# moberweger/deep-prior-pp

Measured on AMD Instinct MI355X. Metric: depth-crops/sec (NYU ResNet50 bs128) 1/2/4/8 GPU; mean 3D joint err (mm), higher is better.
Workload: dtype f32; 1 GPU; NYU posereg_embedding ResNet (type 0, 30-D PCA prior) train step: fused augment + fwd + bwd + ADAM, bs128/GPU fp32, 128x128x1 crops; global_batch=128, parallelism=dp1, augment=True, augment_pipelined=True, bn=local per-GPU batch statistics, launch_mode=native

## Files before the change

### deep-prior-pp_amd/csrc/bn.hip

```cpp
#include "dpp_common.h"

namespace {

constexpr int MAXQ = 256;

template <class TX>
__global__ __launch_bounds__(DPP_THREADS) void bn_stats_partial_kernel(const TX* __restrict__ X, int M, int C,
                                                                       int rpb, float* __restrict__ partial) {
    __shared__ float s_mean[DPP_THREADS * 4];
    __shared__ float s_m2[DPP_THREADS * 4];
    __shared__ float s_n[DPP_THREADS];
    const int Q = C >> 2;
    const int RP = DPP_THREADS / Q;
    const int tid = threadIdx.x;
    const int q = tid % Q, rr = tid / Q;
    const int r_begin = blockIdx.x * rpb;
    const int r_end = (r_begin + rpb < M) ? r_begin + rpb : M;
    float4 K = make_float4(0.f, 0.f, 0.f, 0.f), s1 = K, s2 = K;
    int n = 0;
    if (rr < RP) {
        for (int r = r_begin + rr; r < r_end; r += RP) {
            float4 v = dpp_ld4(X + (size_t)r * C + q * 4);
            if (n == 0) K = v;
            float dx = v.x - K.x, dy = v.y - K.y, dz = v.z - K.z, dw = v.w - K.w;
// ... 15 lines not shown
        for (int j = 0; j < RP; ++j) {
            int t = j * Q + cq;
            double nb = (double)s_n[t];
            if (nb == 0.0) continue;
            double mb = (double)s_mean[t * 4 + ce], m2b = (double)s_m2[t * 4 + ce];
            double delta = mb - mean, tot = cn + nb;
            mean += delta * nb / tot;
            m2 += m2b + delta * delta * cn * nb / tot;
            cn = tot;
        }
        partial[dpp_partial_index(0, c, blockIdx.x, C, gridDim.x)] = (float)mean;
        partial[dpp_partial_index(1, c, blockIdx.x, C, gridDim.x)] = (float)m2;
    }
}

__device__ __forceinline__ double wave_allsum(double v) {
    for (int o = 1; o < DPP_WAVE; o <<= 1) v += __shfl_xor(v, o);
    return v;
}

template <int WPC>
__device__ __forceinline__ double group_allsum(double v, double* slot) {
    v = wave_allsum(v);
    if (WPC == 1) return v;
    const int wave = threadIdx.x >> 6;
    if ((threadIdx.x & 63) == 0) slot[wave] = v;
    __syncthreads();
    return ((slot[0] + slot[1]) + slot[2]) + slot[3];
}

template <int U, int WPC>
__global__ __launch_bounds__(DPP_THREADS) void bn_finalize_kernel(const float* __restrict__ partial, int nbs, int nseg, int M, int rpb,
                                                                  int C, const float* __restrict__ gamma, float eps,
                                                                  float* __restrict__ mean_o, float* __restrict__ inv_std_o,
                                                                  float* __restrict__ scale_o, float* __restrict__ run_mean,
                                                                  float* __restrict__ run_inv_std, float alpha) {
    dpp_kernarg_warm<96>();
    __shared__ double slot_a[4], slot_b[4];
    constexpr int GT = DPP_WAVE * WPC;
    const int lane = threadIdx.x % GT;
    const int c = blockIdx.x * (DPP_THREADS / GT) + threadIdx.x / GT;
    const int cc = c < C ? c : C - 1;
    const bool upd = alpha > 0.0f && run_mean != nullptr;
    const float gam = gamma[cc];
    const float rm_old = (upd ? run_mean : gamma)[cc], ri_old = (upd ? run_inv_std : gamma)[cc];
    const int Mseg = M / nseg;
    auto rows_of = [&](int bi) { return (bi * rpb + rpb <= Mseg) ? rpb : (Mseg - bi * rpb); };
    const bool one_sweep = nseg == 1 && nbs <= GT * U;
    float pm0[U], pq0[U];
    if (one_sweep) {
        const float* pm_row = partial + dpp_partial_index(0, cc, 0, C, nbs);
        const float* pq_row = partial + dpp_partial_index(1, cc, 0, C, nbs);
        const float K = pm_row[0];
#pragma unroll
        for (int u = 0; u < U; ++u) {
            const int b = lane + u * GT;
            const int bb = b < nbs ? b : nbs - 1;
            pm0[u] = pm_row[bb];
            pq0[u] = pq_row[bb];
        }
        double s1 = 0.0, s2 = 0.0;
#pragma unroll
        for (int u = 0; u < U; ++u) {
            const int b = lane + u * GT;
            if (b < nbs) {
                const double d = (double)pm0[u] - (double)K, nb_ = (double)rows_of(b);
                s1 += nb_ * d;
                s2 += (double)pq0[u] + nb_ * d * d;
            }
        }
        s1 = group_allsum<WPC>(s1, slot_a);
        s2 = group_allsum<WPC>(s2, slot_b);
        if (lane != 0 || c >= C) return;
        const double mean1 = (double)K + s1 / (double)M;
        const double var1 = (s2 - s1 * s1 / (double)M) / (double)M;
        const float meanf = (float)mean1;
        const float inv_std = (float)(1.0 / sqrt((var1 > 0.0 ? var1 : 0.0) + (double)eps));
        mean_o[c] = meanf;
        inv_std_o[c] = inv_std;
        scale_o[c] = gam * inv_std;
        if (upd) {
            const float oma = 1.0f - alpha;
            run_mean[c] = oma * rm_old + alpha * meanf;
            run_inv_std[c] = oma * ri_old + alpha * inv_std;
        }
        return;
    }
    double snm = 0.0;
    for (int seg = 0; seg < nseg; ++seg) {
        const float* pm_row = partial + (size_t)seg * 2 * C * nbs + dpp_partial_index(0, cc, 0, C, nbs);
        const float* pq_row = partial + (size_t)seg * 2 * C * nbs + dpp_partial_index(1, cc, 0, C, nbs);
        for (int b0 = lane; b0 < nbs; b0 += GT * U) {
            float pm[U];
#pragma unroll
            for (int u = 0; u < U; ++u) {
                const int b = b0 + u * GT;
                const int bb = b < nbs ? b : nbs - 1;
                pm[u] = pm_row[bb];
            }
#pragma unroll
// ... 443 lines not shown
```

### deep-prior-pp_amd/csrc/gemm.hip

```cpp
#include "gemm_kernels.h"

namespace {

__global__ __launch_bounds__(DPP_THREADS) void reduce_partials_kernel(const float* __restrict__ partial, int nz, int n,
                                                                      const float* __restrict__ bias, int nbias,
                                                                      float* __restrict__ out, int ZL) {
    __shared__ float red[DPP_THREADS];
    const int CB = DPP_THREADS / ZL;
    const int col = threadIdx.x % CB, zl = threadIdx.x / CB;
    for (int i0 = blockIdx.x * CB; i0 < n; i0 += gridDim.x * CB) {
        int i = i0 + col;
        float s = 0.0f;
        if (i < n)
            for (int z = zl; z < nz; z += ZL) s += partial[(size_t)z * n + i];
        if (ZL > 1) {
            red[threadIdx.x] = s;
            __syncthreads();
            if (zl == 0) {
                for (int j = 1; j < ZL; ++j) s += red[j * CB + col];
            }
        }
        if (zl == 0 && i < n) {
            if (bias) s += bias[i % nbias];
            out[i] = s;
// ... 79 lines not shown

bool aligned16(const void* p) { return (reinterpret_cast<uintptr_t>(p) & 15) == 0; }

static int gemm_prepare(const dpp_gemm_desc* dp, GemmArgs& ga) {
    if (!dp || !dp->A || !dp->B || dp->M <= 0 || dp->N <= 0 || dp->K <= 0) return DPP_E_BADARG;
    ga.d = *dp;
    ga.prof = dpp_prof_buffer;
    dpp_gemm_desc& d = ga.d;
    if (d.splitk < 1) d.splitk = 1;
    if (d.splitk > 1 && !d.partial) return DPP_E_BADARG;
    if (d.splitk > 1 && (d.epi.stats || d.epi.bn_x)) return DPP_E_BADARG;
    if (d.epi.bn_x && !(d.epi.bn_mean && d.epi.bn_inv_std && d.epi.bn_scale && d.epi.bn_beta && d.epi.bn_partial)) return DPP_E_BADARG;
    if (d.splitk == 1 && !d.C) return DPP_E_BADARG;
    if (d.actA.mode && d.actA.cmod <= 0) return DPP_E_BADARG;
    if (d.actB.mode && d.actB.cmod <= 0) return DPP_E_BADARG;
    ga.vecA = aligned16(d.A) && (d.lda % 4 == 0);
    if (d.actB.mode & 4) return DPP_E_UNSUPPORTED;
    if (d.actA.mode & 4) {
        if (d.actA.mode != 4 || d.variant == 1 || !d.actA.x2 || !d.actA.aux || !d.actA.mean || !d.actA.scale || !d.actA.beta) return DPP_E_BADARG;
        ga.vecA = ga.vecA && aligned16(d.actA.x2) && aligned16(d.actA.out);
        if (d.actA.out && (!d.a_kc || d.splitk != 1 || d.mapA.s != 1)) return DPP_E_UNSUPPORTED;
        if (!(aligned16(d.actA.mean) && aligned16(d.actA.scale) && aligned16(d.actA.beta) && aligned16(d.actA.aux))) return DPP_E_BADARG;
    }
    ga.vecB = aligned16(d.B) && (d.ldb % 4 == 0);
    if (d.store & ~(DPP_ST_A | DPP_ST_B | DPP_ST_C | DPP_ST_BNX)) return DPP_E_BADARG;
    if (d.precision != 0 && d.precision != 1) return DPP_E_BADARG;
    if (d.precision == 1 && (d.variant == 1 || (d.actA.mode & 4))) return DPP_E_UNSUPPORTED;
    if ((d.store & DPP_ST_A) && (!ga.vecA || (d.actA.mode & 4))) return DPP_E_UNSUPPORTED;
    if ((d.store & DPP_ST_B) && !ga.vecB) return DPP_E_UNSUPPORTED;
    if ((d.store & (DPP_ST_C | DPP_ST_BNX)) && d.splitk != 1) return DPP_E_UNSUPPORTED;
// ... 97 lines not shown
```

### deep-prior-pp_amd/csrc/gemm_expand.hip

```cpp
#include "gemm_args.h"

namespace {

template <int KT, bool BKC, bool IT2, bool ACT, bool RES, bool BNB, bool LZ = false, bool PB = false, bool ST = false>
__global__ __launch_bounds__(DPP_THREADS) DPP_WAVES_PER_EU(1, 2) void gemm_expand_kernel(GemmArgs ga, int rpw) {
    static_assert(!PB || ((KT % 32 == 0 || KT == 16) && !LZ), "bf16 MFMA operands: whole 32-deep steps, or K = 16 with a zero upper half");
    dpp_kernarg_warm<sizeof(GemmArgs)>();
    const dpp_gemm_desc& d = ga.d;
    constexpr int KL = KT / 4, KV = KL / 4;
    constexpr int RT = 2, RI = 16 * RT;
    const int lane = threadIdx.x & 63, l15 = lane & 15, kq = lane >> 4;
    const int NG = d.N >> 6, nblk = d.M / rpw;
    const int gw = blockIdx.x * 4 + (threadIdx.x >> 6);
    if (gw >= NG * nblk) return;
    const int cg = gw % NG, rblk = gw / NG;
    const int n0 = cg * 64 + 4 * l15;
    const int wrow0 = rblk * rpw, iters = rpw / RI;
    const dpp_epilogue& ep = d.epi;
    const int modeA = ACT ? d.actA.mode : 0;
    const bool relu_mask = BNB && ep.bn_relu != 0;
    const bool a16 = ST && !LZ && ga.shA != 0, c16 = ST && (d.store & DPP_ST_C) != 0, x16 = ST && (d.store & DPP_ST_BNX) != 0;
    dpp_stamp(ga.prof, 0);

    float bw[4][KL];
    if (BKC) {
#pragma unroll
        for (int ct = 0; ct < 4; ++ct)
#pragma unroll
            for (int j = 0; j < KV; ++j) {
// ... 33 lines not shown
                    if (LZ) g.a2[rt][j] = *reinterpret_cast<const float4*>(d.actA.x2 + oa + 4 * j);
                }
            }
        }
#pragma unroll
        for (int rt = 0; rt < RT; ++rt)
#pragma unroll
            for (int r = 0; r < 4; ++r) {
                const size_t o = (size_t)(r0 + rt * 16 + kq * 4 + r) * d.ldc + n0;
                if (RES) g.res[rt][r] = c16 ? dpp_raw8(d.residual + (o >> 1)) : *reinterpret_cast<const float4*>(d.residual + o);
                if (BNB) g.bx[rt][r] = x16 ? dpp_raw8(ep.bn_x + (o >> 1)) : *reinterpret_cast<const float4*>(ep.bn_x + o);
            }
    };
    Regs g0, g1;
    fetch(g0, 0);
    float4 mu[KV], sc[KV], be[KV], ax[LZ ? KV : 1];
#pragma unroll
    for (int j = 0; j < KV; ++j) {
        mu[j] = sc[j] = be[j] = make_float4(0.f, 0.f, 0.f, 0.f);
        if (LZ || (modeA & 2)) {
            mu[j] = *reinterpret_cast<const float4*>(d.actA.mean + kq * KL + 4 * j);
            sc[j] = *reinterpret_cast<const float4*>(d.actA.scale + kq * KL + 4 * j);
            be[j] = *reinterpret_cast<const float4*>(d.actA.beta + kq * KL + 4 * j);
        }
        if (LZ) ax[j] = *reinterpret_cast<const float4*>(d.actA.aux + kq * KL + 4 * j);
    }
    const bool lz_store = LZ && d.actA.out != nullptr && cg == 0;
    float4 cbias = make_float4(0.f, 0.f, 0.f, 0.f), cmean = cbias, cscale = cbias, cbeta = cbias, cistd = cbias;
    if (d.bias) cbias = *reinterpret_cast<const float4*>(d.bias + n0);
    if (BNB) {
        cmean = *reinterpret_cast<const float4*>(ep.bn_mean + n0); cscale = *reinterpret_cast<const float4*>(ep.bn_scale + n0);
        cbeta = *reinterpret_cast<const float4*>(ep.bn_beta + n0); cistd = *reinterpret_cast<const float4*>(ep.bn_inv_std + n0);
    }
    dpp_stamp(ga.prof, 1);

    float sx[4] = {0.f, 0.f, 0.f, 0.f}, sy[4] = {0.f, 0.f, 0.f, 0.f};
    float rmean[4] = {0.f, 0.f, 0.f, 0.f}, rm2[4] = {0.f, 0.f, 0.f, 0.f};
    const bool want_stats = ep.stats != nullptr;
    auto colsum = [&](float (&s)[4]) {
#pragma unroll
        for (int j = 0; j < 4; ++j) { s[j] += __shfl_xor(s[j], 16); s[j] += __shfl_xor(s[j], 32); }
    };

    auto step = [&](Regs& g, int it) {
// ... 155 lines not shown
}

}

int dpp_gemm_expand_rows(const dpp_gemm_desc& d, const GemmArgs& ga) {
    if ((d.store & DPP_ST_B) || (d.store && (d.actA.mode & 4))) return 0;
    if (!d.a_kc || d.splitk != 1 || !d.C || !ga.vecA || !ga.vecB || !ga.wide) return 0;
    if (d.K != 16 && d.K != 32 && d.K != 64) return 0;
    if (d.N % 64 || d.M % 32) return 0;
    if (d.mapA.s != 1 || d.mapB.s != 1 || d.mapC.s != 1 || d.actB.mode != 0) return 0;
    if (d.actA.mode != 0 && d.actA.cmod < d.K) return 0;
    if (d.epi.stats && d.epi.bn_x) return 0;
    if (d.b_kc ? (d.epi.bn_x != nullptr || (d.actA.mode & 4)) : (d.actA.mode != 0 && d.actA.mode != 4)) return 0;
    if (d.actA.mode == 4 && d.actA.out && d.lda != d.K) return 0;
    if (d.precision != 0 && (d.precision != 1 || (d.actA.mode & 4))) return 0;
    int rpw = d.bm;
    if (rpw <= 0) rpw = d.M >= 65536 ? 128 : (d.M >= 16384 ? 64 : 32);
    if (rpw % 32 || d.M % rpw) return 0;
    return rpw;
}

namespace {

template <int KT>
int launch_expand(const GemmArgs& ga, int rpw, hipStream_t st) {
    const dpp_gemm_desc& d = ga.d;
    const int waves = (d.M / rpw) * (d.N / 64);
    const dim3 grid(dpp_cdiv(waves, 4));
    const bool it2 = rpw > 32, act = d.actA.mode != 0, res = d.residual != nullptr, bnb = d.epi.bn_x != nullptr, lz = d.actA.mode == 4;
    const bool pb = d.precision == 1;
    const bool stg = d.store != 0;
#define DPP_EXS(K_, I_, A_, R_, B_, L_, P_, S_) DPP_LAUNCH((gemm_expand_kernel<KT, K_, I_, A_, R_, B_, L_, P_, S_>), grid, dim3(DPP_THREADS), 0, st, ga, rpw)
#define DPP_EX(K_, I_, A_, R_, B_, L_, P_) do { if (!(L_) && stg) DPP_EXS(K_, I_, A_, R_, B_, L_, P_, !(L_)); else DPP_EXS(K_, I_, A_, R_, B_, L_, P_, false); } while (0)
#define DPP_EX_P(K_, I_, A_, R_, B_) do { if (pb) { DPP_EX(K_, I_, A_, R_, B_, false, true); break; } \
                                          DPP_EX(K_, I_, A_, R_, B_, false, false); } while (0)
#define DPP_EX_I(K_, A_, R_, B_, L_) do { if (L_) { if (it2) DPP_EX(K_, true, A_, R_, B_, true, false); else DPP_EX(K_, false, A_, R_, B_, true, false); } \
                                          else if (it2) DPP_EX_P(K_, true, A_, R_, B_); else DPP_EX_P(K_, false, A_, R_, B_); } while (0)
#define DPP_EX_R(K_, A_, B_, L_) do { if (res) DPP_EX_I(K_, A_, true, B_, L_); else DPP_EX_I(K_, A_, false, B_, L_); } while (0)
    if (d.b_kc) {
        if (act) DPP_EX_R(true, true, false, false); else DPP_EX_R(true, false, false, false);
    } else if (lz) {
        if (bnb) DPP_EX_R(false, false, true, true); else DPP_EX_R(false, false, false, true);
    } else {
        if (bnb) DPP_EX_R(false, false, true, false); else DPP_EX_R(false, false, false, false);
    }
#undef DPP_EX_P
// ... 14 lines not shown
```

### deep-prior-pp_amd/hipdp/engine.py

```python
import os
from ctypes import c_int as C_int

import numpy as np

from . import evalfuse, layout, ops
from . import heuristics as hz
from .lib import Act, RowMap
from .ops import Plan
from .runtime import default_runtime
from .backward import BackwardMixin
from .store import BNState, ParamStore, TensorV, View, _collect, _dedupe_specs, _layer_kind, _pad4, _param_specs, bf16_bits_to_f32, get_store


class CompiledNet(BackwardMixin):
    def __init__(self, net, train=False, runtime=None, loss=None, weight_decay=0.0, dp=None, fuse_bn=True, bf16=None, optimizer=None,
                 fuse_blocks=None):
        self.rt = rt = runtime or default_runtime()
        self.optimizer = dict(optimizer) if optimizer else dict(name='ADAM')
        self.prec = int(bool(hz.BF16_DEFAULT if bf16 is None else bf16))
        self.store16 = self.grad16 = False
        self.dp = dp
        self.fuse_bn = bool(fuse_bn) and not (dp is not None and dp.sync_bn)
        self.net, self.train = net, train
        self.N = net.cfgParams.batch_size
# ... 265 lines not shown
                return fused

        def fusable(x):
            return x.kind == 'layer' and _layer_kind(x.layer) in ('ConvLayer',) and self._single_consumer(x) \
                and x.layer.cfgParams.activation is None

        cand = [x for x in (a, b) if fusable(x)]
        if not cand:
            raise NotImplementedError("residual add whose operands are not conv outputs")
        q = max(cand, key=lambda x: (self._depth(x) if hz.SIDE_SHORTCUT else 0, x.layer.layerNum))
        p = b if q is a else a
        beside = hz.SIDE_SHORTCUT and self.train and p in cand and id(p) not in self._memo
        if beside:
            self._emit(p.inputs[0])
            n0 = len(self.fwd.ops)
        pv = self._emit(p)
        if not pv.plain:
            raise NotImplementedError("residual add on a non-materialised operand")
        if beside:
            moved = list(self.fwd.ops[n0:])
            if all(isinstance(op, ops.Launch) for op, _ in moved):
                fork = ops.Fork()
                self.fwd.ops[n0:] = [(fork, False)] + [(op, True) for op, _ in moved]
                self.fwd.uses_side = True
                self._emit(q.inputs[0])
                self.fwd.join()
                self._beside.append(([id(fork), id(self.fwd.ops[-1][0])], [id(op) for op, _ in moved]))
        if p.kind == 'layer' and p.layer.layerNum > q.layer.layerNum:
            self._bwd_after[id(p.layer)] = q.layer
        out = self._emit(q, residual=pv.base, out_var=var)
        self._memo[id(q)] = out
# ... 19 lines not shown
        src = self._emit(var.inputs[0])
        if kind == 'BatchNormLayer':
            if not src.plain:
                raise NotImplementedError("BatchNorm on a non-materialised input")
            C = src.base.C
            M = src.base.rows
            sync = self.train and self.dp is not None and self.dp.sync_bn
            b = BNState(layer, C, M, self.dp.world if sync else 1)
            b.mean, b.inv_std, b.scale = (rt.alloc(_pad4(C)) for _ in range(3))
            b.beta_buf, b.gamma_buf = st.view(layer.beta), st.view(layer.gamma)
            b.run_mean, b.run_inv_std = st.view(layer.mean), st.view(layer.inv_std)
            self.bn_states[id(layer)] = b
            fused = getattr(src.base, 'stats', None) if self.train else None
            if fused is not None:
                part, nblk, rows = fused
                self.fwd.add(ops.bn_finalize(rt, part, nblk, M, rows, C, b.gamma_buf, layer.cfgParams.epsilon, b.mean, b.inv_std,
                                             b.scale, b.run_mean, b.run_inv_std, layer.cfgParams.alpha))
            elif self.train:
                W = b.world
                part = self.scratch(b.nb * 2 * C * (W + 1)).view(0, (b.nb * 2 * C,))
                self.fwd.add(ops.bn_stats_partial(rt, src.base.buf, M, C, b.rpb, part))
                if W > 1:
                    allp = self.scratch(b.nb * 2 * C * (W + 1)).view(b.nb * 2 * C, (W * b.nb * 2 * C,))
                    self.fwd.add(self.dp.all_gather_op(part, allp, 'bn_stats_allgather'))
                    part = allp
                self.fwd.add(ops.bn_finalize(rt, part, b.nb, M * W, b.rpb, C, b.gamma_buf, layer.cfgParams.epsilon, b.mean, b.inv_std,
                                             b.scale, b.run_mean, b.run_inv_std, layer.cfgParams.alpha, nseg=W))
            elif hz.EVAL_FUSE:
                self._bn_eval_jobs.append((b.gamma_buf, b.run_mean, b.run_inv_std, C, b.mean, b.inv_std, b.scale))
            else:
                self.fwd.add(ops.bn_eval_coeffs(rt, b.gamma_buf, b.run_mean, b.run_inv_std, C, b.mean, b.inv_std, b.scale))
            v = View(src.base, b, False, shape=src.shape, chan=src.chan)
            v.var = var
            return v
        if kind == 'NonlinearityLayer':
            if layer.cfgParams.activation is None:
                return src
            if layer.cfgParams.activation_str != 'ReLU':
                raise NotImplementedError("only ReLU is on the hot path")
            v = View(src.base, src.bn, True, shape=src.shape, chan=src.chan)
            v.var = var
            return v
        if kind == 'ConvPoolLayer':
            return self._emit_stem(layer, src, out_var if out_var is not None else var)
        if kind == 'ConvLayer':
            return self._emit_conv(layer, src, residual, out_var if out_var is not None else var)
        if kind == 'HiddenLayer':
            return self._emit_fc(layer, src)
        if kind == 'DropoutLayer':
            return self._emit_dropout(layer, src)
        raise NotImplementedError(kind)

    def _emit_stem(self, layer, src, out_var=None):
        c = layer.cfgParams
        N, H, W, Ci = src.base.shape
        ok = (src.base is self.x_in and Ci == 1 and tuple(c.filterDim) == (5, 5) and c.border_mode == 'half' and
              tuple(c.poolsize) == (2, 2) and tuple(c.stride) == (1, 1) and c.activation is None and c.nFilters <= 32)
        if not ok:
            return self._emit_convpool(layer, src)
        Co = c.nFilters
        out = self._new_tensor((N, H // 2, W // 2, Co), 'stem', act=True)
# ... 22 lines not shown
            raise NotImplementedError("'half' padding with an even filter size")
        pad = kh // 2 if c.border_mode == 'half' else 0
        if c.border_mode == 'half' and kh != kw:
            raise NotImplementedError("'half' padding with a non-square filter")
        pool, Co = int(c.poolsize[0]), c.nFilters
        _, Co_, Hp, Wp = c.outputDim
        assert Co_ == Co
        out = self._new_tensor((N, Hp, Wp, Co), 'convpool%d' % layer.layerNum)
        ties = self.rt.alloc((N, Hp, Wp, Co), np.uint16, zero=False) if (self.train and pool > 1) else None
        geom = dict(N=N, H=H, W=W, Ci=Ci, kh=kh, kw=kw, pad=pad, Co=Co, pool=pool, Hp=Hp, Wp=Wp)
        self.fwd.add(ops.convpool_fwd(self.rt, src.base.buf, N, H, W, Ci, self.store.view(layer.W), kh, kw, pad, Co, pool,
                                      self.store.view(layer.b), out.buf, ties, actX=self._act(src), name='convpool_%d' % layer.layerNum))
        self.layer_io[id(layer)] = dict(in_view=src, out=out, ties=ties, geom=geom, stem=False)
        return View(out)

    def _emit_conv(self, layer, src, residual, out_var=None):
        c = layer.cfgParams
        N, Hi, Wi, Ci = src.base.shape
        _, Co, Ho, Wo = c.outputDim
        k, s = tuple(c.filterDim), tuple(c.stride)
        if c.border_mode != 'half' or k not in ((1, 1), (3, 3)) or s[0] != s[1] or (k == (3, 3) and s != (1, 1)):
            raise NotImplementedError("ConvLayer %s stride %s border %s" % (k, s, c.border_mode))
        out = self._new_tensor((N, Ho, Wo, Co), 'conv%d' % layer.layerNum, act=True)
        act = self._act(src)
        rt, st = self.rt, self.store
        res = residual.buf if residual is not None else None
        want_stats = self.train and self.fuse_bn and out_var is not None and self._feeds_batchnorm(out_var)
        M = N * Ho * Wo
        epi = None
        if k == (1, 1):
            tile, _ = hz.gemm_plan(M, Co, Ci, allow_split=False)
            rs = hz.rowstream_plan(M, Co, Ci, True)
            if rs is not None:
                tile = rs
            ks = hz.ksplit_plan(M, Co, Ci) if (s[0] == 1 and rs is None) else None
            if ks is not None:
                tile = ks
            ex = hz.expand_plan(M, Co, Ci, True) if (s[0] == 1 and rs is None and ks is None) else None
            s16 = hz.stream16_plan(M, Co, Ci, True) if (s[0] == 1 and rs is None and ks is None and ex is None) else None
            if s16 is not None:
                tile = s16
            if ex is not None:
                tile = ex
            mp = RowMap.strided(s[0], Ho, Wo, Hi, Wi) if s[0] != 1 else None
            variant = 1 if rs is not None else (2 if ks is not None else (4 if ex is not None else (3 if s16 is not None else 0)))

            def build(tile, variant, epi):
                return ops.gemm(rt, src.base.buf, st.view(layer.W), out.buf, M, Co, Ci, 1, 1, Ci, Ci, Co, mapA=mp, actA=act,
                                bias=st.view(layer.b), residual=res, tile=tile, epi=epi, variant=variant,
                                name='conv1x1_%d' % layer.layerNum, precision=self._gemm_prec(variant, Ci))
            if variant in (2, 3, 4) and ops.gemm_variant_rows(rt, build(tile, variant, None)) != tile[0]:
                variant, (tile, _) = 0, hz.gemm_plan(M, Co, Ci, allow_split=False)
            if want_stats:
                nblk = -(-M // tile[0])
                out.stats = (rt.alloc((nblk, 2, Co), zero=False), nblk, tile[0])
                epi = ops.epilogue(stats=out.stats[0])
            self.fwd.add(build(tile, variant, epi))
        elif self._conv3_stream(N, Hi, Wi, Ci, Co, src.base.buf, out.buf) and residual is None:
            rows = rt.lib.dpp_conv3x3_stream_rows(N, Hi, Wi, Ci)
            if want_stats:
                out.stats = (rt.alloc((M // rows, 2, Co), zero=False), M // rows, rows)
                epi = ops.epilogue(stats=out.stats[0])
            self.fwd.add(ops.conv3x3_stream(rt, src.base.buf, N, Hi, Wi, Ci, st.view(layer.W), out.buf, actX=act, bias=st.view(layer.b), epi=epi,
                                            name='conv3x3_%d' % layer.layerNum))
        else:
            bm = hz.conv3x3_bm(M, Co, hw=(Hi, Wi), prec=self.prec)
            if want_stats:
                th, tw, img = (C_int() for _ in range(3))
                nblk = rt.lib.dpp_conv3x3_tiling(N, Hi, Wi, bm, th, tw, img)
                if Hi % th.value == 0 and Wi % tw.value == 0 and (N % img.value == 0 or nblk == 1):
                    out.stats = (rt.alloc((nblk, 2, Co), zero=False), nblk, bm)
                    epi = ops.epilogue(stats=out.stats[0])
# ... 221 lines not shown
```

### deep-prior-pp_amd/hipdp/heuristics.py

```python
import os

def knob(name, default):
    if os.environ.get('DPP_EXPERIMENT', '0') != '1':
        return default
    return os.environ.get(name, default)


BN_RPB_TARGET_BLOCKS = int(knob('DPP_BN_BLOCKS', '1024'))
BN_BWD_FUSE_MAX_BLOCKS = int(knob('DPP_BN_BWD_FUSE_NB', '0'))
BN_BWD_FUSE_TARGET_WGS = int(knob('DPP_BN_BWD_FUSE_WGS', '512'))



GEMM_TARGET_BLOCKS = int(knob('DPP_GEMM_TARGET_BLOCKS', '1024'))


def gemm_plan(M, N, K, allow_split=True):
    if M <= 16:
        bm, bn, wm = 16, 64, 1
    elif M <= 32:
        bm, bn, wm = 32, 64, 1
    else:
        wm = 4
        cands = [(128, 64), (64, 64), (128, 32), (64, 32), (128, 16), (64, 16)]
        if knob('DPP_NO_128x64', '1') != '0':
# ... 165 lines not shown
```

### deep-prior-pp_amd/hipdp/lib.py

```python
import ctypes as C
import os

_HERE = os.path.dirname(os.path.abspath(__file__))
DEFAULT_LIB = os.path.join(os.path.dirname(_HERE), 'lib', 'libdpp_hip.so')

ABI_VERSION = 24
ST_A, ST_B, ST_C, ST_BNX = 1, 2, 4, 8
c_float_p = C.c_void_p
stream_t = C.c_void_p


class RowMap(C.Structure):
    _fields_ = [('s', C.c_int), ('Wo', C.c_int), ('HoWo', C.c_int), ('Wi', C.c_int), ('HiWi', C.c_int)]

    @staticmethod
    def identity():
        return RowMap(1, 0, 0, 0, 0)

    @staticmethod
    def strided(s, Ho, Wo, Hi, Wi):
        return RowMap(s, Wo, Ho * Wo, Wi, Hi * Wi)


class Act(C.Structure):
    _fields_ = [('mean', C.c_void_p), ('scale', C.c_void_p), ('beta', C.c_void_p), ('mode', C.c_int), ('cmod', C.c_int),
                ('x2', C.c_void_p), ('aux', C.c_void_p), ('out', C.c_void_p)]

    NONE, RELU, BN, BN_RELU, BN_BWD = 0, 1, 2, 3, 4

    @staticmethod
    def none():
        return Act(None, None, None, 0, 1, None, None, None)


class Epilogue(C.Structure):
    _fields_ = [('stats', C.c_void_p), ('bn_x', C.c_void_p), ('bn_mean', C.c_void_p), ('bn_inv_std', C.c_void_p),
                ('bn_scale', C.c_void_p), ('bn_beta', C.c_void_p), ('bn_relu', C.c_int), ('pad_', C.c_int),
                ('bn_partial', C.c_void_p)]


class GemmDesc(C.Structure):
    _fields_ = [('A', C.c_void_p), ('lda', C.c_int), ('a_kc', C.c_int), ('mapA', RowMap), ('actA', Act),
                ('B', C.c_void_p), ('ldb', C.c_int), ('b_kc', C.c_int), ('mapB', RowMap), ('actB', Act),
                ('C', C.c_void_p), ('ldc', C.c_int), ('mapC', RowMap),
                ('bias', C.c_void_p), ('residual', C.c_void_p),
                ('M', C.c_int), ('N', C.c_int), ('K', C.c_int),
                ('splitk', C.c_int), ('partial', C.c_void_p),
                ('bm', C.c_int), ('bn', C.c_int), ('wm', C.c_int), ('variant', C.c_int), ('epi', Epilogue), ('store', C.c_int), ('precision', C.c_int)]


class BnEval(C.Structure):
    _fields_ = [('mean', C.c_void_p), ('inv_std', C.c_void_p), ('gamma', C.c_void_p), ('beta', C.c_void_p)]


class ResblockDesc(C.Structure):
    _fields_ = [('X', C.c_void_p), ('N', C.c_int), ('H', C.c_int), ('W', C.c_int), ('Cin', C.c_int),
                ('stride', C.c_int), ('Ho', C.c_int), ('Wo', C.c_int), ('Cout', C.c_int), ('Nb', C.c_int),
                ('bn0', BnEval), ('bn1', BnEval), ('bn2', BnEval),
                ('W1', C.c_void_p), ('b1', C.c_void_p), ('W2', C.c_void_p), ('b2', C.c_void_p), ('W3', C.c_void_p), ('b3', C.c_void_p),
                ('Wsc', C.c_void_p), ('bsc', C.c_void_p), ('Y', C.c_void_p), ('store', C.c_int)]


SIGNATURES = {
# ... 225 lines not shown
```

### deep-prior-pp_amd/hipdp/ops.py

```python
import ctypes as C
import os

import numpy as np

from .lib import ST_A, ST_B, ST_BNX, ST_C, Act, BnEval, DppError, Epilogue, GemmDesc, ResblockDesc, RowMap, check


class Launch(object):
    __slots__ = ('fn', 'args', 'keep', 'name', 'meta', 'kernels')

    def __init__(self, fn, args, keep, name, meta=None, kernels=1):
        self.fn, self.args, self.keep, self.name, self.meta = fn, args, keep, name, meta
        self.kernels = kernels

    def __call__(self, stream):
        st = self.fn(*self.args, stream)
        if st != 0:
            check(st, self.name)


class Fork(object):
    name = 'fork'
    meta = None

# ... 219 lines not shown
def act_bn_bwd(bn, q, p, x, C, out=None):
    return act(Act.BN_BWD, mean=bn.mean, scale=bn.scale, beta=q, cmod=C, x2=x, aux=p, out=out)


def epilogue(stats=None, bn=None, bn_x=None, bn_relu=True, bn_partial=None):
    e = Epilogue()
    e.stats = _p(stats)
    if bn is not None:
        e.bn_x, e.bn_mean, e.bn_inv_std, e.bn_scale, e.bn_beta = bn_x.ptr, bn.mean.ptr, bn.inv_std.ptr, bn.scale.ptr, bn.beta_buf.ptr
        e.bn_relu, e.bn_partial = int(bn_relu), bn_partial.ptr
    e._bn_x = bn_x
    e._keep = (stats, bn, bn_x, bn_partial)
    return e


def gemm(rt, A, B, Cbuf, M, N, K, a_kc, b_kc, lda, ldb, ldc=0, mapA=None, mapB=None, mapC=None, actA=None, actB=None,
         bias=None, residual=None, splitk=1, partial=None, tile=(0, 0, 0), epi=None, variant=0, name='gemm', precision=0):
    d = GemmDesc()
    d.A, d.lda, d.a_kc = A.ptr, lda, int(a_kc)
    d.mapA = mapA or RowMap.identity()
    d.actA = actA or Act.none()
    d.B, d.ldb, d.b_kc = B.ptr, ldb, int(b_kc)
    d.mapB = mapB or RowMap.identity()
    d.actB = actB or Act.none()
    d.C, d.ldc = _p(Cbuf), ldc
    d.mapC = mapC or RowMap.identity()
    d.bias, d.residual = _p(bias), _p(residual)
    d.M, d.N, d.K = int(M), int(N), int(K)
    d.splitk, d.partial = int(splitk), _p(partial)
    d.bm, d.bn, d.wm = tile
    d.variant = int(variant)
    if epi is not None:
        d.epi = epi
    if _is16(residual) != _is16(Cbuf) and residual is not None and Cbuf is not None:
        raise ValueError("dpp_gemm: C and residual must be stored alike")
    d.store = _store(A, B, Cbuf, getattr(epi, '_bn_x', None) if epi is not None else None)
    d.precision = int(precision)
    meta = dict(kernel='gemm_mfma_bf16' if precision else 'gemm_mfma_f32', flops=2.0 * M * N * K,
                bytes=_esz(A) * M * K + _esz(B) * K * N + (4.0 * M * N * max(1, splitk) if splitk > 1 else _esz(Cbuf) * M * N) +
                (_esz(residual) * M * N if residual is not None else 0))
    return Launch(rt.lib.dpp_gemm, (C.byref(d),), (d, A, B, Cbuf, bias, residual, partial, actA, actB, epi), name, meta)


def gemm_variant_rows(rt, launch):
    return int(rt.lib.dpp_gemm_variant_rows(C.byref(launch.keep[0])))


def wgrad_stream(rt, dY, Co, X, Ci, M, rows_per_wave, partial, mapX=None, actX=None, name='wgrad_stream', precision=0):
    nsl = rt.lib.dpp_wgrad_stream_slices(Co, Ci, M, rows_per_wave)
    meta = dict(kernel='gemm_mfma_bf16' if precision else 'gemm_mfma_f32', flops=2.0 * M * Co * Ci,
                bytes=_esz(dY) * M * Co + 4.0 * nsl * Co * Ci + _esz(X) * M * Ci)
    return Launch(rt.lib.dpp_wgrad_stream_bf16 if precision else rt.lib.dpp_wgrad_stream, (dY.ptr, int(Co), X.ptr, int(Ci), C.byref(mapX) if mapX is not None else None, _actp(actX), int(M),
                                            int(rows_per_wave), partial.ptr, _store(a=dY, b=X)), (dY, X, partial, mapX, actX), name, meta)


def wgrad3_stream(rt, dY, Co, X, Ci, N, H, W, rows_per_wave, partial, actX=None, name='conv3x3_wgrad_stream'):
# ... 966 lines not shown
```

### include/dpp_hip.h

```cpp
#ifndef DPP_HIP_H
#define DPP_HIP_H

#include <stddef.h>
#include <stdint.h>

#ifdef __cplusplus
extern "C" {
#endif

typedef void* dpp_stream_t;

#define DPP_OK 0
#define DPP_E_BADARG 10001
#define DPP_E_UNSUPPORTED 10002

#define DPP_ABI_VERSION 24
int dpp_abi_version(void);

#define DPP_ST_A 1
#define DPP_ST_B 2
#define DPP_ST_C 4
#define DPP_ST_BNX 8

typedef struct {
    int s, Wo, HoWo, Wi, HiWi;
} dpp_rowmap;

typedef struct {
    const float* mean;
    const float* scale;
    const float* beta;
// ... 3 lines not shown
    const float* aux;
    float* out;
} dpp_act;

typedef struct {
    float* stats;
    const float* bn_x;
    const float* bn_mean;
    const float* bn_inv_std;
    const float* bn_scale;
    const float* bn_beta;
    int bn_relu;
    int pad_;
    float* bn_partial;
} dpp_epilogue;

typedef struct {
    const float* A; int lda; int a_kc; dpp_rowmap mapA; dpp_act actA;
    const float* B; int ldb; int b_kc; dpp_rowmap mapB; dpp_act actB;
    float* C; int ldc; dpp_rowmap mapC;
    const float* bias;
    const float* residual;
    int M, N, K;
    int splitk;
    float* partial;
    int bm, bn, wm;
    int variant;
    dpp_epilogue epi;
    int store;
    int precision;
} dpp_gemm_desc;
int dpp_gemm(const dpp_gemm_desc* d, dpp_stream_t stream);
int dpp_gemm_variant_rows(const dpp_gemm_desc* d);
int dpp_gemm_walk_grid(const dpp_gemm_desc* d, int* gx, int* gy);

int dpp_wgrad_stream_slices(int Co, int Ci, int M, int rows_per_wave);
int dpp_wgrad_stream(const float* dY, int Co, const float* X, int Ci, const dpp_rowmap* mapX, const dpp_act* actX, int M,
                     int rows_per_wave, float* partial, int store , dpp_stream_t stream);
int dpp_wgrad_stream_bf16_ok(int Co, int Ci);
int dpp_wgrad_stream_bf16(const float* dY, int Co, const float* X, int Ci, const dpp_rowmap* mapX, const dpp_act* actX, int M,
                     int rows_per_wave, float* partial, int store , dpp_stream_t stream);

int dpp_fc_wgrad_stream_ok(int Nb, int K, int N);
int dpp_fc_wgrad_stream(const float* X, const float* dY, float* dW, int Nb, int K, int N, const dpp_act* actX,
                        int store , dpp_stream_t stream);
// ... 314 lines not shown
```

Baseline: 38310 depth-crops/sec.

## Fold BatchNorm finalize into the consuming expand GEMM prologue

For small-channel BatchNorm layers feeding a 1x1 expand GEMM, each workgroup now reduces the per-block partial statistics itself and derives mean/scale/beta into shared memory. The separate bn_finalize launch is then dropped from the forward op list. Block 0 writes the mean, inv_std, scale and running statistics to global memory. This removes one kernel launch and a serialization point per eligible layer, at the cost of every workgroup redundantly re-reading the partials (bounded by size heuristics) and a new ABI field in the GEMM descriptor.

```diff
diff --git a/deep-prior-pp_amd/csrc/bn.hip b/deep-prior-pp_amd/csrc/bn.hip
--- a/deep-prior-pp_amd/csrc/bn.hip
+++ b/deep-prior-pp_amd/csrc/bn.hip
@@ -1,4 +1,5 @@
 #include "dpp_common.h"
+#include "bn_finalize.h"
 
 namespace {
 
@@ -53,14 +54,9 @@
     }
 }
 
-__device__ __forceinline__ double wave_allsum(double v) {
-    for (int o = 1; o < DPP_WAVE; o <<= 1) v += __shfl_xor(v, o);
-    return v;
-}
-
 template <int WPC>
 __device__ __forceinline__ double group_allsum(double v, double* slot) {
-    v = wave_allsum(v);
+    v = dpp_wave_allsum(v);
     if (WPC == 1) return v;
     const int wave = threadIdx.x >> 6;
     if ((threadIdx.x & 63) == 0) slot[wave] = v;
@@ -86,43 +82,12 @@
     const int Mseg = M / nseg;
     auto rows_of = [&](int bi) { return (bi * rpb + rpb <= Mseg) ? rpb : (Mseg - bi * rpb); };
     const bool one_sweep = nseg == 1 && nbs <= GT * U;
-    float pm0[U], pq0[U];
     if (one_sweep) {
-        const float* pm_row = partial + dpp_partial_index(0, cc, 0, C, nbs);
-        const float* pq_row = partial + dpp_partial_index(1, cc, 0, C, nbs);
-        const float K = pm_row[0];
-#pragma unroll
-        for (int u = 0; u < U; ++u) {
-            const int b = lane + u * GT;
-            const int bb = b < nbs ? b : nbs - 1;
-            pm0[u] = pm_row[bb];
-            pq0[u] = pq_row[bb];
-        }
-        double s1 = 0.0, s2 = 0.0;
-#pragma unroll
-        for (int u = 0; u < U; ++u) {
-            const int b = lane + u * GT;
-            if (b < nbs) {
-                const double d = (double)pm0[u] - (double)K, nb_ = (double)rows_of(b);
-                s1 += nb_ * d;
-                s2 += (double)pq0[u] + nb_ * d * d;
-            }
-        }
-        s1 = group_allsum<WPC>(s1, slot_a);
-        s2 = group_allsum<WPC>(s2, slot_b);
+        const dpp_bn_sums sums = dpp_bn_finalize_sweep<U, GT>(partial + dpp_partial_index(0, cc, 0, C, nbs), partial + dpp_partial_index(1, cc, 0, C, nbs),
+                                                              lane, nbs, rpb, M, [&](double v) { return group_allsum<WPC>(v, slot_a); },
+                                                              [&](double v) { return group_allsum<WPC>(v, slot_b); });
         if (lane != 0 || c >= C) return;
-        const double mean1 = (double)K + s1 / (double)M;
-        const double var1 = (s2 - s1 * s1 / (double)M) / (double)M;
-        const float meanf = (float)mean1;
-        const float inv_std = (float)(1.0 / sqrt((var1 > 0.0 ? var1 : 0.0) + (double)eps));
-        mean_o[c] = meanf;
-        inv_std_o[c] = inv_std;
-        scale_o[c] = gam * inv_std;
-        if (upd) {
-            const float oma = 1.0f - alpha;
-            run_mean[c] = oma * rm_old + alpha * meanf;
-            run_inv_std[c] = oma * ri_old + alpha * inv_std;
-        }
+        dpp_bn_finalize_store(dpp_bn_finalize_coef(sums, M, eps, gam), c, mean_o, inv_std_o, scale_o, upd, run_mean, run_inv_std, rm_old, ri_old, alpha);
         return;
     }
     double snm = 0.0;
diff --git a/deep-prior-pp_amd/csrc/bn_finalize.h b/deep-prior-pp_amd/csrc/bn_finalize.h
--- /dev/null
+++ b/deep-prior-pp_amd/csrc/bn_finalize.h
@@ -0,0 +1,86 @@
+#pragma once
+#include "dpp_common.h"
+
+struct dpp_bn_sums { double K, s1, s2; };
+struct dpp_bn_coef { float mean, inv_std, scale; };
+
+template <int U, int GT, class SumA, class SumB>
+__device__ __forceinline__ dpp_bn_sums dpp_bn_finalize_sweep(const float* __restrict__ pm_row, const float* __restrict__ pq_row, int lane, int nbs,
+                                                             int rpb, int M, SumA sum_a, SumB sum_b) {
+#pragma clang fp contract(off)
+    float pm0[U], pq0[U];
+    const float K = pm_row[0];
+#pragma unroll
+    for (int u = 0; u < U; ++u) {
+        const int b = lane + u * GT;
+        const int bb = b < nbs ? b : nbs - 1;
+        pm0[u] = pm_row[bb];
+        pq0[u] = pq_row[bb];
+    }
+    double s1 = 0.0, s2 = 0.0;
+#pragma unroll
+    for (int u = 0; u < U; ++u) {
+        const int b = lane + u * GT;
+        if (b < nbs) {
+            const double d = (double)pm0[u] - (double)K;
+            const double nb_ = (double)((b * rpb + rpb <= M) ? rpb : (M - b * rpb));
+            const double nd = nb_ * d;
+            s1 = __builtin_fma(nb_, d, s1);
+            s2 = s2 + __builtin_fma(nd, d, (double)pq0[u]);
+        }
+    }
+    dpp_bn_sums r;
+    r.K = (double)K;
+    r.s1 = sum_a(s1);
+    r.s2 = sum_b(s2);
+    return r;
+}
+
+__device__ __forceinline__ dpp_bn_coef dpp_bn_finalize_coef(const dpp_bn_sums& s, int M, float eps, float gam) {
+#pragma clang fp contract(off)
+    const double mean1 = s.K + s.s1 / (double)M;
+    const double var1 = (s.s2 - s.s1 * s.s1 / (double)M) / (double)M;
+    dpp_bn_coef r;
+    r.mean = (float)mean1;
+    r.inv_std = (float)(1.0 / sqrt((var1 > 0.0 ? var1 : 0.0) + (double)eps));
+    r.scale = gam * r.inv_std;
+    return r;
+}
+
+__device__ __forceinline__ void dpp_bn_finalize_store(const dpp_bn_coef& k, int c, float* __restrict__ mean_o, float* __restrict__ inv_std_o,
+                                                      float* __restrict__ scale_o, bool upd, float* __restrict__ run_mean,
+                                                      float* __restrict__ run_inv_std, float rm_old, float ri_old, float alpha) {
+#pragma clang fp contract(off)
+    mean_o[c] = k.mean;
+    inv_std_o[c] = k.inv_std;
+    scale_o[c] = k.scale;
+    if (upd) {
+        const float oma = 1.0f - alpha;
+        run_mean[c] = oma * rm_old + alpha * k.mean;
+        run_inv_std[c] = oma * ri_old + alpha * k.inv_std;
+    }
+}
+
+__device__ __forceinline__ double dpp_wave_allsum(double v) {
+    for (int o = 1; o < DPP_WAVE; o <<= 1) v += __shfl_xor(v, o);
+    return v;
+}
+
+template <int N>
+__device__ __forceinline__ double dpp_wave_allsum_split(double (&v)[N], int lane) {
+    static_assert(N >= 1 && N <= DPP_WAVE && (N & (N - 1)) == 0, "a power of two of vectors");
+    int o = 1;
+#pragma unroll
+    for (int n = N; n > 1; n >>= 1, o <<= 1) {
+        const bool hi = (lane & o) != 0;
+#pragma unroll
+        for (int j = 0; j < n / 2; ++j) {
+            const double keep = hi ? v[2 * j + 1] : v[2 * j], send = hi ? v[2 * j] : v[2 * j + 1];
+            v[j] = keep + __shfl_xor(send, o);
+        }
+    }
+    double r = v[0];
+#pragma unroll
+    for (; o < DPP_WAVE; o <<= 1) r += __shfl_xor(r, o);
+    return r;
+}
diff --git a/deep-prior-pp_amd/csrc/gemm.hip b/deep-prior-pp_amd/csrc/gemm.hip
--- a/deep-prior-pp_amd/csrc/gemm.hip
+++ b/deep-prior-pp_amd/csrc/gemm.hip
@@ -117,6 +117,12 @@
     if (d.splitk == 1 && !d.C) return DPP_E_BADARG;
     if (d.actA.mode && d.actA.cmod <= 0) return DPP_E_BADARG;
     if (d.actB.mode && d.actB.cmod <= 0) return DPP_E_BADARG;
+    if (d.derive.partial) {
+        const dpp_bn_derive& v = d.derive;
+        if (!v.gamma || !v.mean || !v.inv_std || !v.scale || v.nb < 1 || v.rows_per_block < 1 || v.M < 1 || v.nb != dpp_cdiv(v.M, v.rows_per_block) ||
+            (v.run_mean != nullptr) != (v.run_inv_std != nullptr)) return DPP_E_BADARG;
+        if (d.variant != 4) return DPP_E_UNSUPPORTED;
+    }
     ga.vecA = aligned16(d.A) && (d.lda % 4 == 0);
     if (d.actB.mode & 4) return DPP_E_UNSUPPORTED;
     if (d.actA.mode & 4) {
diff --git a/deep-prior-pp_amd/csrc/gemm_expand.hip b/deep-prior-pp_amd/csrc/gemm_expand.hip
--- a/deep-prior-pp_amd/csrc/gemm_expand.hip
+++ b/deep-prior-pp_amd/csrc/gemm_expand.hip
@@ -1,18 +1,58 @@
 #include "gemm_args.h"
+#include "bn_finalize.h"
 
 namespace {
 
-template <int KT, bool BKC, bool IT2, bool ACT, bool RES, bool BNB, bool LZ = false, bool PB = false, bool ST = false>
+template <int KT>
+__device__ __forceinline__ void expand_derive_coefs(const dpp_bn_derive& dv, const float* __restrict__ beta, float* s_coef, int lane) {
+    constexpr int CPW = KT / 4;
+    const int wave = threadIdx.x >> 6;
+    auto sweep = [&](auto utag) {
+        constexpr int U = decltype(utag)::value;
+        constexpr int CH = (32 / U) < CPW ? (32 / U) : CPW;
+        auto own = [](double v) { return v; };
+        for (int c0 = wave * CPW; c0 < (wave + 1) * CPW; c0 += CH) {
+            const int c = c0 + (lane & (CH - 1));
+            const bool writer = blockIdx.x == 0 && lane < CH, upd = writer && dv.alpha > 0.0f && dv.run_mean != nullptr;
+            const float gam = dv.gamma[c], bet = beta[c], piv = dv.partial[dpp_partial_index(0, c, 0, KT, dv.nb)];
+            const float rm_old = (upd ? dv.run_mean : dv.gamma)[c], ri_old = (upd ? dv.run_inv_std : dv.gamma)[c];
+            double s1[CH], s2[CH];
+#pragma unroll
+            for (int i = 0; i < CH; ++i) {
+                const dpp_bn_sums t = dpp_bn_finalize_sweep<U, DPP_WAVE>(dv.partial + dpp_partial_index(0, c0 + i, 0, KT, dv.nb),
+                                                                         dv.partial + dpp_partial_index(1, c0 + i, 0, KT, dv.nb), lane, dv.nb,
+                                                                         dv.rows_per_block, dv.M, own, own);
+                s1[i] = t.s1;
+                s2[i] = t.s2;
+            }
+            dpp_bn_sums sums;
+            sums.K = (double)piv;
+            sums.s1 = dpp_wave_allsum_split<CH>(s1, lane);
+            sums.s2 = dpp_wave_allsum_split<CH>(s2, lane);
+            const dpp_bn_coef co = dpp_bn_finalize_coef(sums, dv.M, dv.eps, gam);
+            if (lane < CH) { s_coef[c] = co.mean; s_coef[KT + c] = co.scale; s_coef[2 * KT + c] = bet; }
+            if (writer) dpp_bn_finalize_store(co, c, dv.mean, dv.inv_std, dv.scale, upd, dv.run_mean, dv.run_inv_std, rm_old, ri_old, dv.alpha);
+        }
+    };
+    if (dv.nb <= 2 * DPP_WAVE) sweep(std::integral_constant<int, 2>());
+    else if (dv.nb <= 4 * DPP_WAVE) sweep(std::integral_constant<int, 4>());
+    else sweep(std::integral_constant<int, 8>());
+}
+
+template <int KT, bool BKC, bool IT2, bool ACT, bool RES, bool BNB, bool LZ = false, bool PB = false, bool ST = false, bool DRV = false>
 __global__ __launch_bounds__(DPP_THREADS) DPP_WAVES_PER_EU(1, 2) void gemm_expand_kernel(GemmArgs ga, int rpw) {
     static_assert(!PB || ((KT % 32 == 0 || KT == 16) && !LZ), "bf16 MFMA operands: whole 32-deep steps, or K = 16 with a zero upper half");
+    static_assert(!DRV || (BKC && ACT && !BNB && !LZ && !PB && !ST), "derived BatchNorm coefficients: the forward float32 form only");
     dpp_kernarg_warm<sizeof(GemmArgs)>();
     const dpp_gemm_desc& d = ga.d;
     constexpr int KL = KT / 4, KV = KL / 4;
     constexpr int RT = 2, RI = 16 * RT;
     const int lane = threadIdx.x & 63, l15 = lane & 15, kq = lane >> 4;
     const int NG = d.N >> 6, nblk = d.M / rpw;
-    const int gw = blockIdx.x * 4 + (threadIdx.x >> 6);
-    if (gw >= NG * nblk) return;
+    const int gw_ = blockIdx.x * 4 + (threadIdx.x >> 6);
+    const bool live = gw_ < NG * nblk;
+    if (!DRV && !live) return;
+    const int gw = (DRV && !live) ? 0 : gw_;
     const int cg = gw % NG, rblk = gw / NG;
     const int n0 = cg * 64 + 4 * l15;
     const int wrow0 = rblk * rpw, iters = rpw / RI;
@@ -76,9 +116,22 @@
     };
     Regs g0, g1;
     fetch(g0, 0);
-    float4 mu[KV], sc[KV], be[KV], ax[LZ ? KV : 1];
-#pragma unroll
-    for (int j = 0; j < KV; ++j) {
+    float4 mu[KV], sc[KV], be[KV], ax[LZ ? KV : 1], bias_d = make_float4(0.f, 0.f, 0.f, 0.f);
+    if (DRV) {
+        __shared__ float s_coef[3 * KT];
+        if (d.bias) bias_d = *reinterpret_cast<const float4*>(d.bias + n0);
+        expand_derive_coefs<KT>(d.derive, d.actA.beta, s_coef, lane);
+        __syncthreads();
+        if (!live) return;
+#pragma unroll
+        for (int j = 0; j < KV; ++j) {
+            mu[j] = *reinterpret_cast<const float4*>(&s_coef[kq * KL + 4 * j]);
+            sc[j] = *reinterpret_cast<const float4*>(&s_coef[KT + kq * KL + 4 * j]);
+            be[j] = *reinterpret_cast<const float4*>(&s_coef[2 * KT + kq * KL + 4 * j]);
+        }
+    }
+#pragma unroll
+    for (int j = 0; j < (DRV ? 0 : KV); ++j) {
         mu[j] = sc[j] = be[j] = make_float4(0.f, 0.f, 0.f, 0.f);
         if (LZ || (modeA & 2)) {
             mu[j] = *reinterpret_cast<const float4*>(d.actA.mean + kq * KL + 4 * j);
@@ -89,7 +142,8 @@
     }
     const bool lz_store = LZ && d.actA.out != nullptr && cg == 0;
     float4 cbias = make_float4(0.f, 0.f, 0.f, 0.f), cmean = cbias, cscale = cbias, cbeta = cbias, cistd = cbias;
-    if (d.bias) cbias = *reinterpret_cast<const float4*>(d.bias + n0);
+    if (DRV) cbias = bias_d;
+    else if (d.bias) cbias = *reinterpret_cast<const float4*>(d.bias + n0);
     if (BNB) {
         cmean = *reinterpret_cast<const float4*>(ep.bn_mean + n0); cscale = *reinterpret_cast<const float4*>(ep.bn_scale + n0);
         cbeta = *reinterpret_cast<const float4*>(ep.bn_beta + n0); cistd = *reinterpret_cast<const float4*>(ep.bn_inv_std + n0);
@@ -275,6 +329,7 @@
     if (d.b_kc ? (d.epi.bn_x != nullptr || (d.actA.mode & 4)) : (d.actA.mode != 0 && d.actA.mode != 4)) return 0;
     if (d.actA.mode == 4 && d.actA.out && d.lda != d.K) return 0;
     if (d.precision != 0 && (d.precision != 1 || (d.actA.mode & 4))) return 0;
+    if (d.derive.partial && (!d.b_kc || !(d.actA.mode & 2) || !d.actA.beta || d.precision != 0 || d.store != 0 || d.derive.nb > 8 * DPP_WAVE)) return 0;
     int rpw = d.bm;
     if (rpw <= 0) rpw = d.M >= 65536 ? 128 : (d.M >= 16384 ? 64 : 32);
     if (rpw % 32 || d.M % rpw) return 0;
@@ -291,6 +346,13 @@
     const bool it2 = rpw > 32, act = d.actA.mode != 0, res = d.residual != nullptr, bnb = d.epi.bn_x != nullptr, lz = d.actA.mode == 4;
     const bool pb = d.precision == 1;
     const bool stg = d.store != 0;
+    if (d.derive.partial) {
+#define DPP_EXD(I_, R_) DPP_LAUNCH((gemm_expand_kernel<KT, true, I_, true, R_, false, false, false, false, true>), grid, dim3(DPP_THREADS), 0, st, ga, rpw)
+        if (it2) { if (res) DPP_EXD(true, true); else DPP_EXD(true, false); }
+        else { if (res) DPP_EXD(false, true); else DPP_EXD(false, false); }
+#undef DPP_EXD
+        return dpp_launch_status();
+    }
 #define DPP_EXS(K_, I_, A_, R_, B_, L_, P_, S_) DPP_LAUNCH((gemm_expand_kernel<KT, K_, I_, A_, R_, B_, L_, P_, S_>), grid, dim3(DPP_THREADS), 0, st, ga, rpw)
 #define DPP_EX(K_, I_, A_, R_, B_, L_, P_) do { if (!(L_) && stg) DPP_EXS(K_, I_, A_, R_, B_, L_, P_, !(L_)); else DPP_EXS(K_, I_, A_, R_, B_, L_, P_, false); } while (0)
 #define DPP_EX_P(K_, I_, A_, R_, B_) do { if (pb) { DPP_EX(K_, I_, A_, R_, B_, false, true); break; } \
diff --git a/deep-prior-pp_amd/hipdp/engine.py b/deep-prior-pp_amd/hipdp/engine.py
--- a/deep-prior-pp_amd/hipdp/engine.py
+++ b/deep-prior-pp_amd/hipdp/engine.py
@@ -303,7 +303,9 @@
         if beside:
             self._emit(p.inputs[0])
             n0 = len(self.fwd.ops)
+        self._beside_now = beside
         pv = self._emit(p)
+        self._beside_now = False
         if not pv.plain:
             raise NotImplementedError("residual add on a non-materialised operand")
         if beside:
@@ -353,8 +355,9 @@
             fused = getattr(src.base, 'stats', None) if self.train else None
             if fused is not None:
                 part, nblk, rows = fused
-                self.fwd.add(ops.bn_finalize(rt, part, nblk, M, rows, C, b.gamma_buf, layer.cfgParams.epsilon, b.mean, b.inv_std,
-                                             b.scale, b.run_mean, b.run_inv_std, layer.cfgParams.alpha))
+                fin = self.fwd.add(ops.bn_finalize(rt, part, nblk, M, rows, C, b.gamma_buf, layer.cfgParams.epsilon, b.mean, b.inv_std,
+                                                   b.scale, b.run_mean, b.run_inv_std, layer.cfgParams.alpha))
+                b.finalize = (fin, var, part, nblk, rows)
             elif self.train:
                 W = b.world
                 part = self.scratch(b.nb * 2 * C * (W + 1)).view(0, (b.nb * 2 * C,))
@@ -383,7 +386,7 @@
         if kind == 'ConvPoolLayer':
             return self._emit_stem(layer, src, out_var if out_var is not None else var)
         if kind == 'ConvLayer':
-            return self._emit_conv(layer, src, residual, out_var if out_var is not None else var)
+            return self._emit_conv(layer, src, residual, out_var if out_var is not None else var, in_var=var.inputs[0])
         if kind == 'HiddenLayer':
             return self._emit_fc(layer, src)
         if kind == 'DropoutLayer':
@@ -436,7 +439,34 @@
         self.layer_io[id(layer)] = dict(in_view=src, out=out, ties=ties, geom=geom, stem=False)
         return View(out)
 
-    def _emit_conv(self, layer, src, residual, out_var=None):
+    def _bn_derive(self, src, in_var, variant, prec, takes):
+        b = src.bn
+        fin = getattr(b, 'finalize', None) if b is not None else None
+        if fin is None or not self.train or variant != 4 or prec != 0 or src.base.is16 or in_var is None or getattr(self, '_beside_now', False):
+            return None
+        op, bn_var, part, nblk, rows = fin
+        if not hz.bn_derive_ok(nblk, b.C) or not any(o is op for o, _ in self.fwd.ops):
+            return None
+        v = in_var
+        while True:
+            if not self._single_consumer(v):
+                return None
+            if v is bn_var:
+                break
+            if v.kind == 'relu' or (v.kind == 'layer' and _layer_kind(v.layer) == 'NonlinearityLayer'):
+                v = v.inputs[0]
+            else:
+                return None
+        c = b.layer.cfgParams
+        dv = ops.bn_derive(part, nblk, b.M, rows, b.gamma_buf, c.epsilon, b.mean, b.inv_std, b.scale, b.run_mean, b.run_inv_std, c.alpha)
+        if not takes(dv):
+            return None
+        self.fwd.ops = [(o, side) for (o, side) in self.fwd.ops if o is not op]
+        b.finalize = None
+        b.derived = True
+        return dv
+
+    def _emit_conv(self, layer, src, residual, out_var=None, in_var=None):
         c = layer.cfgParams
         N, Hi, Wi, Ci = src.base.shape
         _, Co, Ho, Wo = c.outputDim
@@ -467,17 +497,19 @@
             mp = RowMap.strided(s[0], Ho, Wo, Hi, Wi) if s[0] != 1 else None
             variant = 1 if rs is not None else (2 if ks is not None else (4 if ex is not None else (3 if s16 is not None else 0)))
 
-            def build(tile, variant, epi):
+            def build(tile, variant, epi, derive=None):
                 return ops.gemm(rt, src.base.buf, st.view(layer.W), out.buf, M, Co, Ci, 1, 1, Ci, Ci, Co, mapA=mp, actA=act,
                                 bias=st.view(layer.b), residual=res, tile=tile, epi=epi, variant=variant,
-                                name='conv1x1_%d' % layer.layerNum, precision=self._gemm_prec(variant, Ci))
+                                name='conv1x1_%d' % layer.layerNum, precision=self._gemm_prec(variant, Ci), derive=derive)
             if variant in (2, 3, 4) and ops.gemm_variant_rows(rt, build(tile, variant, None)) != tile[0]:
                 variant, (tile, _) = 0, hz.gemm_plan(M, Co, Ci, allow_split=False)
             if want_stats:
                 nblk = -(-M // tile[0])
                 out.stats = (rt.alloc((nblk, 2, Co), zero=False), nblk, tile[0])
                 epi = ops.epilogue(stats=out.stats[0])
-            self.fwd.add(build(tile, variant, epi))
+            dv = self._bn_derive(src, in_var, variant, self._gemm_prec(variant, Ci),
+                                 lambda dv: ops.gemm_variant_rows(rt, build(tile, variant, epi, dv)) == tile[0])
+            self.fwd.add(build(tile, variant, epi, dv))
         elif self._conv3_stream(N, Hi, Wi, Ci, Co, src.base.buf, out.buf) and residual is None:
             rows = rt.lib.dpp_conv3x3_stream_rows(N, Hi, Wi, Ci)
             if want_stats:
diff --git a/deep-prior-pp_amd/hipdp/heuristics.py b/deep-prior-pp_amd/hipdp/heuristics.py
--- a/deep-prior-pp_amd/hipdp/heuristics.py
+++ b/deep-prior-pp_amd/hipdp/heuristics.py
@@ -9,6 +9,14 @@
 BN_RPB_TARGET_BLOCKS = int(knob('DPP_BN_BLOCKS', '1024'))
 BN_BWD_FUSE_MAX_BLOCKS = int(knob('DPP_BN_BWD_FUSE_NB', '0'))
 BN_BWD_FUSE_TARGET_WGS = int(knob('DPP_BN_BWD_FUSE_WGS', '512'))
+BN_DERIVE = knob('DPP_BN_DERIVE', '1') != '0'
+BN_DERIVE_MAX_BYTES = int(knob('DPP_BN_DERIVE_BYTES', str(64 << 10)))
+BN_DERIVE_MAX_CHANNELS = int(knob('DPP_BN_DERIVE_CHANNELS', '32'))
+BN_DERIVE_MAX_BLOCKS = 512
+
+
+def bn_derive_ok(nb, C):
+    return BN_DERIVE and nb <= BN_DERIVE_MAX_BLOCKS and C <= BN_DERIVE_MAX_CHANNELS and 8 * nb * C <= BN_DERIVE_MAX_BYTES
 
 
 
diff --git a/deep-prior-pp_amd/hipdp/lib.py b/deep-prior-pp_amd/hipdp/lib.py
--- a/deep-prior-pp_amd/hipdp/lib.py
+++ b/deep-prior-pp_amd/hipdp/lib.py
@@ -4,7 +4,7 @@
 _HERE = os.path.dirname(os.path.abspath(__file__))
 DEFAULT_LIB = os.path.join(os.path.dirname(_HERE), 'lib', 'libdpp_hip.so')
 
-ABI_VERSION = 24
+ABI_VERSION = 25
 ST_A, ST_B, ST_C, ST_BNX = 1, 2, 4, 8
 c_float_p = C.c_void_p
 stream_t = C.c_void_p
@@ -37,6 +37,12 @@
     _fields_ = [('stats', C.c_void_p), ('bn_x', C.c_void_p), ('bn_mean', C.c_void_p), ('bn_inv_std', C.c_void_p),
                 ('bn_scale', C.c_void_p), ('bn_beta', C.c_void_p), ('bn_relu', C.c_int), ('pad_', C.c_int),
                 ('bn_partial', C.c_void_p)]
+
+
+class BnDerive(C.Structure):
+    _fields_ = [('partial', C.c_void_p), ('nb', C.c_int), ('rows_per_block', C.c_int), ('M', C.c_int), ('eps', C.c_float),
+                ('gamma', C.c_void_p), ('alpha', C.c_float), ('pad_', C.c_int), ('run_mean', C.c_void_p), ('run_inv_std', C.c_void_p),
+                ('mean', C.c_void_p), ('inv_std', C.c_void_p), ('scale', C.c_void_p)]
 
 
 class GemmDesc(C.Structure):
@@ -46,7 +52,8 @@
                 ('bias', C.c_void_p), ('residual', C.c_void_p),
                 ('M', C.c_int), ('N', C.c_int), ('K', C.c_int),
                 ('splitk', C.c_int), ('partial', C.c_void_p),
-                ('bm', C.c_int), ('bn', C.c_int), ('wm', C.c_int), ('variant', C.c_int), ('epi', Epilogue), ('store', C.c_int), ('precision', C.c_int)]
+                ('bm', C.c_int), ('bn', C.c_int), ('wm', C.c_int), ('variant', C.c_int), ('epi', Epilogue), ('store', C.c_int), ('precision', C.c_int),
+                ('pad_', C.c_int), ('derive', BnDerive)]
 
 
 class BnEval(C.Structure):
diff --git a/deep-prior-pp_amd/hipdp/ops.py b/deep-prior-pp_amd/hipdp/ops.py
--- a/deep-prior-pp_amd/hipdp/ops.py
+++ b/deep-prior-pp_amd/hipdp/ops.py
@@ -3,7 +3,7 @@
 
 import numpy as np
 
-from .lib import ST_A, ST_B, ST_BNX, ST_C, Act, BnEval, DppError, Epilogue, GemmDesc, ResblockDesc, RowMap, check
+from .lib import ST_A, ST_B, ST_BNX, ST_C, Act, BnDerive, BnEval, DppError, Epilogue, GemmDesc, ResblockDesc, RowMap, check
 
 
 class Launch(object):
@@ -257,8 +257,17 @@
     return e
 
 
+def bn_derive(partial, nb, M, rpb, gamma, eps, mean, inv_std, scale, run_mean=None, run_inv_std=None, alpha=0.0):
+    v = BnDerive()
+    v.partial, v.nb, v.rows_per_block, v.M, v.eps = partial.ptr, int(nb), int(rpb), int(M), float(eps)
+    v.gamma, v.alpha, v.run_mean, v.run_inv_std = gamma.ptr, float(alpha), _p(run_mean), _p(run_inv_std)
+    v.mean, v.inv_std, v.scale = mean.ptr, inv_std.ptr, scale.ptr
+    v._keep = (partial, gamma, mean, inv_std, scale, run_mean, run_inv_std)
+    return v
+
+
 def gemm(rt, A, B, Cbuf, M, N, K, a_kc, b_kc, lda, ldb, ldc=0, mapA=None, mapB=None, mapC=None, actA=None, actB=None,
-         bias=None, residual=None, splitk=1, partial=None, tile=(0, 0, 0), epi=None, variant=0, name='gemm', precision=0):
+         bias=None, residual=None, splitk=1, partial=None, tile=(0, 0, 0), epi=None, variant=0, name='gemm', precision=0, derive=None):
     d = GemmDesc()
     d.A, d.lda, d.a_kc = A.ptr, lda, int(a_kc)
     d.mapA = mapA or RowMap.identity()
@@ -279,10 +288,12 @@
         raise ValueError("dpp_gemm: C and residual must be stored alike")
     d.store = _store(A, B, Cbuf, getattr(epi, '_bn_x', None) if epi is not None else None)
     d.precision = int(precision)
+    if derive is not None:
+        d.derive = derive
     meta = dict(kernel='gemm_mfma_bf16' if precision else 'gemm_mfma_f32', flops=2.0 * M * N * K,
                 bytes=_esz(A) * M * K + _esz(B) * K * N + (4.0 * M * N * max(1, splitk) if splitk > 1 else _esz(Cbuf) * M * N) +
                 (_esz(residual) * M * N if residual is not None else 0))
-    return Launch(rt.lib.dpp_gemm, (C.byref(d),), (d, A, B, Cbuf, bias, residual, partial, actA, actB, epi), name, meta)
+    return Launch(rt.lib.dpp_gemm, (C.byref(d),), (d, A, B, Cbuf, bias, residual, partial, actA, actB, epi, derive), name, meta)
 
 
 def gemm_variant_rows(rt, launch):
diff --git a/include/dpp_hip.h b/include/dpp_hip.h
--- a/include/dpp_hip.h
+++ b/include/dpp_hip.h
@@ -14,7 +14,7 @@
 #define DPP_E_BADARG 10001
 #define DPP_E_UNSUPPORTED 10002
 
-#define DPP_ABI_VERSION 24
+#define DPP_ABI_VERSION 25
 int dpp_abi_version(void);
 
 #define DPP_ST_A 1
@@ -48,6 +48,20 @@
     int pad_;
     float* bn_partial;
 } dpp_epilogue;
+
+typedef struct {
+    const float* partial;
+    int nb, rows_per_block, M;
+    float eps;
+    const float* gamma;
+    float alpha;
+    int pad_;
+    float* run_mean;
+    float* run_inv_std;
+    float* mean;
+    float* inv_std;
+    float* scale;
+} dpp_bn_derive;
 
 typedef struct {
     const float* A; int lda; int a_kc; dpp_rowmap mapA; dpp_act actA;
@@ -63,6 +77,8 @@
     dpp_epilogue epi;
     int store;
     int precision;
+    int pad_;
+    dpp_bn_derive derive;
 } dpp_gemm_desc;
 int dpp_gemm(const dpp_gemm_desc* d, dpp_stream_t stream);
 int dpp_gemm_variant_rows(const dpp_gemm_desc* d);
```

Result: no change. 38450 depth-crops/sec, median of 6 (+0.4%).
